# grantneale/kafka-lag-based-assignor

Hardware: AMD Instinct MI355X
Metric: partition-assignments/sec (whole node) (higher is better)
Workload: dtype int64

## Files before the change

kafka_lag_based_assignor_amd/csrc/la_device.h:

```cpp
#pragma once
#include <hip/hip_runtime.h>
#include <stdint.h>

namespace la {

constexpr int kWave = 64;

struct Rec {
    uint32_t hi, lo, tb;
};

__device__ __forceinline__ bool rec_less(const Rec& a, const Rec& b) {
    const uint64_t ka = ((uint64_t)a.hi << 32) | a.lo;
    const uint64_t kb = ((uint64_t)b.hi << 32) | b.lo;
    return (ka < kb) | ((ka == kb) & (a.tb < b.tb));
}

__device__ __forceinline__ int64_t partition_lag(int64_t begin, int64_t end, int64_t committed,
                                                 bool reset_latest) {
    const int64_t next = committed >= 0 ? committed : (reset_latest ? end : begin);
    const int64_t d = (int64_t)((uint64_t)end - (uint64_t)next);
    return d > 0 ? d : 0;
}

// ... 15 lines not shown
        return (uint32_t)__builtin_amdgcn_mov_dpp((int)x, 0x128, 0xF, 0xF, false);
    } else if constexpr (J == 16) {
        auto r = __builtin_amdgcn_permlane16_swap(x, x, false, false);
        return (__lane_id() & 16) ? r[0] : r[1];
    } else {
        auto r = __builtin_amdgcn_permlane32_swap(x, x, false, false);
        return (__lane_id() & 32) ? r[0] : r[1];
    }
}

template <int J>
__device__ __forceinline__ Rec shfl_xor(const Rec& r) {
    Rec o;
    o.hi = shfl_xor<J>(r.hi);
    o.lo = shfl_xor<J>(r.lo);
    o.tb = shfl_xor<J>(r.tb);
    return o;
}

__device__ __forceinline__ Rec shfl_xor_dyn(const Rec& r, int j) {
    switch (j) {
        case 1: return shfl_xor<1>(r);
        case 2: return shfl_xor<2>(r);
        case 4: return shfl_xor<4>(r);
        case 8: return shfl_xor<8>(r);
        case 16: return shfl_xor<16>(r);
        default: return shfl_xor<32>(r);
    }
}

template <int J>
__device__ __forceinline__ void cmpx_lanes(Rec& mine, bool keep_min) {
    const Rec o = shfl_xor<J>(mine);
    const bool take = (rec_less(o, mine) == keep_min);
    mine.hi = take ? o.hi : mine.hi;
    mine.lo = take ? o.lo : mine.lo;
    mine.tb = take ? o.tb : mine.tb;
}

__device__ __forceinline__ void cmpx_lanes_dyn(Rec& mine, int j, bool keep_min) {
    const Rec o = shfl_xor_dyn(mine, j);
    const bool take = (rec_less(o, mine) == keep_min);
    mine.hi = take ? o.hi : mine.hi;
    mine.lo = take ? o.lo : mine.lo;
    mine.tb = take ? o.tb : mine.tb;
}

__device__ __forceinline__ void cmpx_regs(Rec& a, Rec& b, bool asc) {
    const bool sw = (rec_less(b, a) == asc);
    const Rec ta = a, tb_ = b;
    a.hi = sw ? tb_.hi : ta.hi;  a.lo = sw ? tb_.lo : ta.lo;  a.tb = sw ? tb_.tb : ta.tb;
    b.hi = sw ? ta.hi : tb_.hi;  b.lo = sw ? ta.lo : tb_.lo;  b.tb = sw ? ta.tb : tb_.tb;
}

template <int L, int E, int K, int J>
__device__ __forceinline__ void bitonic_stage(Rec (&rec)[E], int gl) {
    constexpr int N = L * E;
    if constexpr (J >= E) {
        constexpr int JL = J / E;
        const bool lower = (gl & JL) == 0;
        const bool asc = (K == N) ? true : ((gl & (K / E)) == 0);
        const bool keep_min = (lower == asc);
#pragma unroll
        for (int r = 0; r < E; ++r) cmpx_lanes<JL>(rec[r], keep_min);
    } else {
#pragma unroll
        for (int r = 0; r < E; ++r) {
            if ((r & J) == 0) {
                bool asc;
                if constexpr (K == N) asc = true;
                else if constexpr (K < E) asc = ((r & K) == 0);
                else asc = ((gl & (K / E)) == 0);
                cmpx_regs(rec[r], rec[r | J], asc);
            }
        }
    }
}

template <int L, int E, int K, int J>
__device__ __forceinline__ void bitonic_merge(Rec (&rec)[E], int gl) {
    bitonic_stage<L, E, K, J>(rec, gl);
    if constexpr (J > 1) bitonic_merge<L, E, K, J / 2>(rec, gl);
}

template <int L, int E, int K = 2>
__device__ __forceinline__ void bitonic_sort_tile(Rec (&rec)[E], int gl) {
    if constexpr (L * E >= 2) {
        bitonic_merge<L, E, K, K / 2>(rec, gl);
        if constexpr (K < L * E) bitonic_sort_tile<L, E, K * 2>(rec, gl);
    }
}

__device__ __forceinline__ void bitonic_sort_lanes(Rec& rec, int gl, int n) {
    for (int k = 2; k <= n; k <<= 1) {
        for (int j = k >> 1; j > 0; j >>= 1) {
            const bool keep_min = (((gl & j) == 0) == ((gl & k) == 0));
            cmpx_lanes_dyn(rec, j, keep_min);
        }
    }
}


__device__ __forceinline__ uint32_t dpp_row_mirror(uint32_t x) {
    return (uint32_t)__builtin_amdgcn_mov_dpp((int)x, 0x140, 0xF, 0xF, false);
}

template <int M>
__device__ __forceinline__ uint32_t shfl_mirror(uint32_t x) {
    static_assert(M == 2 || M == 4 || M == 8 || M == 16 || M == 32 || M == 64, "bad mirror width");
    if constexpr (M == 2) return shfl_xor<1>(x);
    else if constexpr (M == 4) return (uint32_t)__builtin_amdgcn_mov_dpp((int)x, 0x1B, 0xF, 0xF, false);
    else if constexpr (M == 8) return (uint32_t)__builtin_amdgcn_mov_dpp((int)x, 0x141, 0xF, 0xF, false);
    else if constexpr (M == 16) return dpp_row_mirror(x);
    else if constexpr (M == 32) return shfl_xor<16>(dpp_row_mirror(x));
    else return shfl_xor<32>(shfl_xor<16>(dpp_row_mirror(x)));
}

__device__ __forceinline__ uint32_t wave_or_u32(uint32_t v) {
    v |= shfl_xor<1>(v);
    v |= shfl_xor<2>(v);
    v |= shfl_xor<4>(v);
    v |= shfl_xor<8>(v);
    v |= shfl_xor<16>(v);
    v |= shfl_xor<32>(v);
    return v;
}

__device__ __forceinline__ void wave_lds_fence() {
    __builtin_amdgcn_fence(__ATOMIC_RELEASE, "wavefront");
    __builtin_amdgcn_wave_barrier();
    __builtin_amdgcn_fence(__ATOMIC_ACQUIRE, "wavefront");
}

__device__ __forceinline__ void lds_barrier() {
    asm volatile("s_waitcnt lgkmcnt(0)\n\ts_barrier" ::: "memory");
}

__device__ __forceinline__ uint32_t wave_incl_scan_u32(uint32_t v) {
    v += (uint32_t)__builtin_amdgcn_update_dpp(0, (int)v, 0x111, 0xF, 0xF, false);
    v += (uint32_t)__builtin_amdgcn_update_dpp(0, (int)v, 0x112, 0xF, 0xF, false);
    v += (uint32_t)__builtin_amdgcn_update_dpp(0, (int)v, 0x114, 0xF, 0xF, false);
    v += (uint32_t)__builtin_amdgcn_update_dpp(0, (int)v, 0x118, 0xF, 0xF, false);
    v += (uint32_t)__builtin_amdgcn_update_dpp(0, (int)v, 0x142, 0xA, 0xF, false);
    v += (uint32_t)__builtin_amdgcn_update_dpp(0, (int)v, 0x143, 0xC, 0xF, false);
    return v;
}

__device__ __forceinline__ int wave_max_i32(int v) {
#pragma unroll
    for (int d = 32; d >= 1; d >>= 1) v = max(v, __shfl_xor(v, d));
    return v;
}

}
```

kafka_lag_based_assignor_amd/csrc/la_sort64.h:

```cpp
#pragma once
#include <hip/hip_runtime.h>
#include <stdint.h>

#include "la_device.h"

namespace la {

struct P64 {
    uint32_t lo, hi;
};

__device__ __forceinline__ P64 p64_from(uint64_t x) { P64 p; p.lo = (uint32_t)x; p.hi = (uint32_t)(x >> 32); return p; }
__device__ __forceinline__ uint64_t p64_value(const P64& p) { return ((uint64_t)p.hi << 32) | p.lo; }

template <int J>
struct KeepMin {
    static_assert(J == 1 || J == 2 || J == 4 || J == 8 || J == 16 || J == 32, "bad lane bit");
    static constexpr uint64_t value = J == 1 ? 0x5555555555555555ull : J == 2 ? 0x3333333333333333ull
                                    : J == 4 ? 0x0F0F0F0F0F0F0F0Full : J == 8 ? 0x00FF00FF00FF00FFull
                                    : J == 16 ? 0x0000FFFF0000FFFFull : 0x00000000FFFFFFFFull;
};

#define LA_DPP_TAIL " row_mask:0xf bank_mask:0xf"
#define LA_FIX_S(K) "s_xor_b64 vcc, vcc, " K "\n\t"
// ... 99 lines not shown
                 "v_cndmask_b32 %0, %3, %0, vcc\n\t"             \
                 "v_cndmask_b32 %1, %4, %1, vcc"                 \
                 : "+v"(r.lo), "+v"(r.hi), "=&v"(t)              \
                 : "v"(o.lo), "v"(o.hi), KC(KV)                  \
                 : "vcc", "scc")
template <int J, bool VO = false>
__device__ __forceinline__ void select_minmax(P64& r, const P64& o) {
    uint32_t t;
    if constexpr (VO) {
        const uint32_t kvec = keep_vec<J>();
        LA_SELECT_ASM(LA_FIX_V("%2", "%5"), "v", kvec);
    } else {
        const uint64_t keep = KeepMin<J>::value;
        LA_SELECT_ASM(LA_FIX_S("%5"), "s", keep);
    }
}

template <int M, int PAD, bool VO = false>
__device__ __forceinline__ void cmpx_same_mirror(P64& r) {
    static_assert(M == 2 || M == 4 || M == 8 || M == 16 || M == 32 || M == 64, "bad mirror width");
    if constexpr (M == 2) {
        cmpx_same_xor<1, PAD, VO>(r);
    } else if constexpr (M == 4 || M == 8 || M == 16) {
        [[maybe_unused]] const uint64_t keep = KeepMin<M / 2>::value;
        [[maybe_unused]] const uint32_t kvec = keep_vec<M / 2>();
        uint32_t t;
        if constexpr (M == 4) LA_SAME_PADS("quad_perm:[3,2,1,0]");
        else if constexpr (M == 8) LA_SAME_PADS("row_half_mirror");
        else LA_SAME_PADS("row_mirror");
    } else {
        asm volatile("s_nop 1" : "+v"(r.lo), "+v"(r.hi));
        P64 o;
        o.lo = shfl_mirror<M>(r.lo);
        o.hi = shfl_mirror<M>(r.hi);
        select_minmax<M / 2, VO>(r, o);
    }
}

#define LA_CROSS_ASM(PADSTR, CTRL, FIX, KC, KV)                                             \
    asm volatile(PADSTR                                                                     \
                 "v_sub_co_u32_dpp %2, vcc, %0, %5 " CTRL LA_DPP_TAIL "\n\t"                  \
                 "v_subb_co_u32_dpp %2, vcc, %1, %6, vcc " CTRL LA_DPP_TAIL "\n\t"            \
                 FIX                                                                        \
                 "v_cndmask_b32_dpp %3, %0, %5, vcc " CTRL LA_DPP_TAIL "\n\t"                 \
                 "v_cndmask_b32_dpp %4, %1, %6, vcc " CTRL LA_DPP_TAIL "\n\t"                 \
                 "v_sub_co_u32_dpp %2, vcc, %5, %0 " CTRL LA_DPP_TAIL "\n\t"                  \
                 "v_subb_co_u32_dpp %2, vcc, %6, %1, vcc " CTRL LA_DPP_TAIL "\n\t"            \
                 FIX                                                                        \
                 "v_cndmask_b32_dpp %0, %5, %0, vcc " CTRL LA_DPP_TAIL "\n\t"                 \
                 "v_cndmask_b32_dpp %1, %6, %1, vcc " CTRL LA_DPP_TAIL                        \
                 : "+v"(q.lo), "+v"(q.hi), "=&v"(t), "=&v"(n.lo), "=&v"(n.hi)                       \
                 : "v"(r.lo), "v"(r.hi), KC(KV)                                             \
                 : "vcc", "scc")
#define LA_CROSS_VO(PADSTR, CTRL)                                                          \
    do {                                                                                   \
        if constexpr (VO) LA_CROSS_ASM(PADSTR, CTRL, LA_FIX_V("%2", "%7"), "v", kvec);     \
        else LA_CROSS_ASM(PADSTR, CTRL, LA_FIX_S("%7"), "s", keep);                        \
    } while (0)

#define LA_CROSS_PADS(CTRL)                                   \
    do {                                                      \
        if constexpr (PAD == 0) LA_CROSS_VO(LA_PAD0, CTRL);    \
        else if constexpr (PAD == 1) LA_CROSS_VO(LA_PAD1, CTRL); \
        else LA_CROSS_VO(LA_PAD2, CTRL);                       \
    } while (0)

template <int M, int PAD, bool VO = false>
__device__ __forceinline__ void cmpx_cross_mirror(P64& r, P64& q) {
    static_assert(M == 2 || M == 4 || M == 8 || M == 16 || M == 32 || M == 64, "bad mirror width");
    [[maybe_unused]] const uint64_t keep = KeepMin<M / 2>::value;
    [[maybe_unused]] const uint32_t kvec = keep_vec<M / 2>();
    if constexpr (M <= 16) {
        uint32_t t;
        P64 n;
        if constexpr (M == 2) LA_CROSS_PADS("quad_perm:[1,0,3,2]");
        else if constexpr (M == 4) LA_CROSS_PADS("quad_perm:[3,2,1,0]");
        else if constexpr (M == 8) LA_CROSS_PADS("row_half_mirror");
        else LA_CROSS_PADS("row_mirror");
        r = n;
    } else {
        asm volatile("s_nop 1" : "+v"(r.lo), "+v"(r.hi), "+v"(q.lo), "+v"(q.hi));
        P64 oq, orr;
        oq.lo = shfl_mirror<M>(q.lo); oq.hi = shfl_mirror<M>(q.hi);
        orr.lo = shfl_mirror<M>(r.lo); orr.hi = shfl_mirror<M>(r.hi);
        select_minmax<M / 2, VO>(r, oq);
        select_minmax<M / 2, VO>(q, orr);
    }
}

__device__ __forceinline__ void cmpx_regs_p64(P64& a, P64& b) {
    uint32_t t;
    P64 n;
    asm volatile("v_sub_co_u32 %2, vcc, %0, %5\n\t"
                 "v_subb_co_u32 %2, vcc, %1, %6, vcc\n\t"
                 "v_cndmask_b32 %3, %5, %0, vcc\n\t"
                 "v_cndmask_b32 %4, %6, %1, vcc\n\t"
                 "v_cndmask_b32 %0, %0, %5, vcc\n\t"
                 "v_cndmask_b32 %1, %1, %6, vcc"
                 : "+v"(b.lo), "+v"(b.hi), "=&v"(t), "=&v"(n.lo), "=&v"(n.hi)
                 : "v"(a.lo), "v"(a.hi)
                 : "vcc", "scc");
    a = n;
}


template <int L, int E, int J, bool FIRST, bool VO = false>
__device__ __forceinline__ void clean_p64(P64 (&rec)[E]) {
    if constexpr (J >= 1) {
        if constexpr (J >= E) {
            constexpr int PADN = (E <= 2) ? 1 : 0;
#pragma unroll
            for (int r = 0; r < E; ++r) cmpx_same_xor<J / E, PADN, VO>(rec[r]);
        } else {
#pragma unroll
            for (int r = 0; r < E; ++r)
                if ((r & J) == 0) cmpx_regs_p64(rec[r], rec[r | J]);
        }
        clean_p64<L, E, J / 2, false, VO>(rec);
    }
}

template <int L, int E, int K, bool FIRST, bool VO = false>
__device__ __forceinline__ void merge_p64(P64 (&rec)[E]) {
    if constexpr (K <= L * E) {
        if constexpr (K <= E) {
#pragma unroll
            for (int r = 0; r < E; ++r)
                if ((r & (K >> 1)) == 0) cmpx_regs_p64(rec[r], rec[r ^ (K - 1)]);
        } else {
            constexpr int M = K / E;
            if constexpr (E == 1) {
                cmpx_same_mirror<M, FIRST ? 2 : 1, VO>(rec[0]);
            } else {
                constexpr int PADN = FIRST ? 2 : ((E <= 2) ? 1 : 0);
#pragma unroll
                for (int r = E / 2 - 1; r >= 0; --r) cmpx_cross_mirror<M, PADN, VO>(rec[r], rec[E - 1 - r]);
            }
        }
        clean_p64<L, E, K / 4, false, VO>(rec);
        merge_p64<L, E, K * 2, false, VO>(rec);
    }
}

template <int L, int E, bool VO = false>
__device__ __forceinline__ void bitonic_sort_tile_p64(P64 (&rec)[E]) {
    if constexpr (E == 1) merge_p64<L, E, 2, true, VO>(rec);
    else merge_p64<L, E, 2, false, VO>(rec);
}


__device__ __forceinline__ uint64_t p64_of_prev_lane(const P64& r) {
    const uint32_t lo = (uint32_t)__builtin_amdgcn_update_dpp(0, (int)r.lo, 0x138, 0xF, 0xF, false);
    const uint32_t hi = (uint32_t)__builtin_amdgcn_update_dpp(0, (int)r.hi, 0x138, 0xF, 0xF, false);
    return ((uint64_t)hi << 32) | lo;
}

__device__ __forceinline__ bool lanes_in_order_p64(const P64& r, int gl) {
    const uint64_t prev = p64_of_prev_lane(r);
    const bool bad = (gl > 0) & (prev > p64_value(r));
    return __builtin_amdgcn_ballot_w64(bad) == 0;
}

template <int L, bool VO = false>
__device__ __forceinline__ void bitonic_sort_lanes_p64(P64& rec) {
    P64 r1[1] = {rec};
    merge_p64<L, 1, 2, true, VO>(r1);
    rec = r1[0];
}

#define LA_R_STEP(CTRL, KEEP)                                                         \
    "v_sub_co_u32_dpp %[t], vcc, %[lo], %[lo] " CTRL LA_DPP_TAIL "\n\t"               \
    "v_subb_co_u32_dpp %[t], vcc, %[hi], %[hi], vcc " CTRL LA_DPP_TAIL "\n\t"         \
    "v_xor_b32 %[t], %[" KEEP "], %[t]\n\t"                                          \
    "v_cmp_gt_i32 vcc, 0, %[t]\n\t"                                                  \
    "v_cndmask_b32_dpp %[lo], %[lo], %[lo], vcc " CTRL LA_DPP_TAIL "\n\t"             \
    "v_cndmask_b32_dpp %[hi], %[hi], %[hi], vcc " CTRL LA_DPP_TAIL "\n\t"
#define LA_R_STEP_X4(KEEP)                                                                     \
    "v_mov_b32_dpp %[u], %[lo] row_half_mirror" LA_DPP_TAIL "\n\t"                               \
    "v_mov_b32_dpp %[w], %[hi] row_half_mirror" LA_DPP_TAIL "\n\t"                               \
    "s_nop 0\n\t"                                                                              \
    "v_sub_co_u32_dpp %[t], vcc, %[u], %[lo] quad_perm:[3,2,1,0]" LA_DPP_TAIL "\n\t"             \
    "v_subb_co_u32_dpp %[t], vcc, %[w], %[hi], vcc quad_perm:[3,2,1,0]" LA_DPP_TAIL "\n\t"       \
    "v_xor_b32 %[t], %[" KEEP "], %[t]\n\t"                                                   \
    "v_cmp_gt_i32 vcc, 0, %[t]\n\t"                                                           \
    "v_cndmask_b32_dpp %[lo], %[u], %[lo], vcc quad_perm:[3,2,1,0]" LA_DPP_TAIL "\n\t"           \
    "v_cndmask_b32_dpp %[hi], %[w], %[hi], vcc quad_perm:[3,2,1,0]" LA_DPP_TAIL "\n\t"
#define LA_R_X1 "quad_perm:[1,0,3,2]"
#define LA_R_X2 "quad_perm:[2,3,0,1]"
#define LA_R_M4 "quad_perm:[3,2,1,0]"
#define LA_R_NOP "s_nop 0\n\t"
#define LA_R_ADV "v_add_u32 %[sb], %[stride], %[sb]\n\t"
#define LA_R_CLAMP "v_min_u32 %[abn], %[zb], %[sb]\n\t"
#define LA_R_READ "ds_read_b64 %[nxt], %[abn]\n\t"
#define LA_R_TAIL                                            \
    "s_waitcnt lgkmcnt(0)\n\t"                               \
    "v_add_co_u32 %[lo], vcc, %[clo], %[lo]\n\t"             \
    "v_addc_co_u32 %[hi], vcc, %[chi], %[hi], vcc\n\t"       \
    "v_and_b32 %[won], %[mk], %[lo]\n\t"                     \
    "ds_write_b32 %[abc], %[won]"
#define LA_R_NET2 LA_R_STEP(LA_R_X1, "k1")
#define LA_R_NET4_REST LA_R_STEP(LA_R_M4, "k2") LA_R_CLAMP LA_R_STEP(LA_R_X1, "k1")
#define LA_R_NET8_REST LA_R_STEP("row_half_mirror", "k4") LA_R_NOP LA_R_STEP(LA_R_X2, "k2") LA_R_NOP LA_R_STEP(LA_R_X1, "k1")
#define LA_R_NET16_REST \
    LA_R_STEP("row_mirror", "k8") LA_R_NOP LA_R_STEP_X4("k4") LA_R_NOP LA_R_STEP(LA_R_X2, "k2") LA_R_NOP LA_R_STEP(LA_R_X1, "k1")
#define LA_ROUND_ASM(BODY)                                                                                             \
    asm volatile(BODY LA_R_TAIL                                                                                        \
                 : [lo] "+v"(bin.lo), [hi] "+v"(bin.hi), [sb] "+v"(sb), [abn] "=&v"(ab_next), [nxt] "=&v"(nxt),         \
                   [t] "=&v"(t), [u] "=&v"(u), [w] "=&v"(w), [won] "=&v"(won)                                           \
                 : [abc] "v"(ab_cur), [clo] "v"((uint32_t)cur), [chi] "v"((uint32_t)(cur >> 32)), [stride] "s"(stride), \
                   [zb] "s"(zb), [mk] "v"(lane_mask), [k1] "v"(kv[0]), [k2] "v"(kv[1]), [k4] "v"(kv[2]), [k8] "v"(kv[3]) \
                 : "vcc", "memory")

constexpr uint64_t kRoundSentinel = 0x7FFFFFFFFFFFFFFFull;

__device__ __forceinline__ void round_keep_vectors(int lane, uint32_t (&kv)[4]) {
#pragma unroll
    for (int b = 0; b < 4; ++b) kv[b] = (lane & (1 << b)) ? 0u : 0xFFFFFFFFu;
}

template <int L>
__device__ __forceinline__ void greedy_round_p64(P64& bin, uint32_t& sb, uint32_t ab_cur, uint32_t& ab_next, uint64_t cur,
                                                 uint64_t& nxt, uint32_t stride, uint32_t zb, uint32_t lane_mask,
                                                 const uint32_t (&kv)[4]) {
    static_assert(L == 2 || L == 4 || L == 8 || L == 16, "one statement per width up to a DPP row");
    uint32_t t, u, w, won;
    if constexpr (L == 2) LA_ROUND_ASM(LA_R_ADV LA_R_CLAMP LA_R_READ LA_R_NET2);
    else if constexpr (L == 4) LA_ROUND_ASM(LA_R_ADV LA_R_NET2 LA_R_CLAMP LA_R_STEP(LA_R_M4, "k2") LA_R_READ LA_R_STEP(LA_R_X1, "k1"));
    else if constexpr (L == 8) LA_ROUND_ASM(LA_R_NET2 LA_R_ADV LA_R_NET4_REST LA_R_READ LA_R_NET8_REST);
    else LA_ROUND_ASM(LA_R_NET2 LA_R_ADV LA_R_NET4_REST LA_R_READ LA_R_NET8_REST LA_R_NOP LA_R_NET16_REST);
}

}
```

kafka_lag_based_assignor_amd/csrc/la_wave_tile_impl.h:

```cpp
#pragma once
#include "la_kernels.h"
#include "la_device.h"
#include "la_sort64.h"
#include "la_sort32.h"
#include "la_group_small.h"
#ifdef LA_LAB
#include <cstdio>
#include <cstdlib>
#endif

namespace la {

enum : int { kModeAuto = 0, kModeWide = 1, kModeArgmin = 2 };

#ifndef LA_ABLATE
#define LA_ABLATE 0
#endif
constexpr int kAblate = LA_ABLATE;
#ifndef LA_SKIP_SORTED_ROUNDS
#define LA_SKIP_SORTED_ROUNDS 1
#endif
constexpr bool kSkipSortedRounds = LA_SKIP_SORTED_ROUNDS != 0;
#ifndef LA_WPB
#define LA_WPB 4
// ... 94 lines not shown
#pragma unroll
    for (int k = 0; k < NP; ++k) {
        const auto g = clamped_index<L, E, FULL>(a, d, 2 * k, gl);
        if constexpr (E >= 2) {
            raw.en[k] = load_at<I64x2>(src_en, g);
            raw.id[k] = load_at<I32x2>(a.pid, g);
        } else {
            raw.en[k].x = load_at<int64_t>(src_en, g); raw.en[k].y = 0;
            raw.id[k].x = load_at<int32_t>(a.pid, g); raw.id[k].y = 0;
        }
    }
}

template <int L, int E>
__device__ __forceinline__ bool second_stage_needed(const TileArgs& a) {
    return !a.lag && !a.reset_latest && a.begin;
}

template <int L, int E, bool FULL = false, typename D>
__device__ __forceinline__ void issue_begin_loads(const TileArgs& a, const D& d, int gl, Raw<E>& raw) {
    if constexpr (kAblate == 2) return;
    constexpr int NP = (E + 1) / 2;
    if (!second_stage_needed<L, E>(a)) return;
    {
        bool any = false;
#pragma unroll
        for (int k = 0; k < NP; ++k) any |= (raw.cm[k].x < 0) | (E >= 2 && raw.cm[k].y < 0);
        if (__builtin_amdgcn_ballot_w64(any) == 0 && !(a.flags & kTileAlwaysStage2)) return;
    }
#pragma unroll
    for (int k = 0; k < NP; ++k) {
        const auto g = clamped_index<L, E, FULL>(a, d, 2 * k, gl);
        using G = decltype(g);
        const bool nx = raw.cm[k].x < 0;
        if constexpr (E >= 2) {
            const bool ny = raw.cm[k].y < 0;
            const I64x2 bv = load_at<I64x2>(a.begin, (nx | ny) ? g : (G)0);
            raw.cm[k].x = nx ? bv.x : raw.cm[k].x;
            raw.cm[k].y = ny ? bv.y : raw.cm[k].y;
        } else {
            const int64_t vx = a.begin[nx ? g : (G)0];
            raw.cm[k].x = nx ? vx : raw.cm[k].x;
        }
    }
}

template <int L, int E, bool FULL = false, typename D>
__device__ __forceinline__ void finish_lags(const TileArgs& a, const D& d, int gl, const Raw<E>& raw,
                                            int64_t (&lag)[E], int32_t (&pid)[E]) {
    const bool latest = a.reset_latest != 0;
    if constexpr (kAblate == 2) {
#pragma unroll
        for (int v = 0; v < E; ++v) {
            const uint32_t h = ((uint32_t)d.p0 + (uint32_t)(v * L + gl)) * 2654435761u;
            lag[v] = (int64_t)(h >> 2) + a.reset_latest;
            pid[v] = (int32_t)((v * L + gl) * 77 + 13) & (L * E - 1);
        }
        return;
    }
    constexpr int NP = (E + 1) / 2;
    const bool cm_is_next = second_stage_needed<L, E>(a);
    auto lag_of = [&](int64_t en, int64_t cm) -> int64_t {
        if (a.lag) return en;
        if (cm_is_next) { const int64_t dlt = (int64_t)((uint64_t)en - (uint64_t)cm); return dlt > 0 ? dlt : 0; }
        return partition_lag(0, en, cm, latest);
    };
#pragma unroll
    for (int k = 0; k < NP; ++k) {
        const int e = load_index<L, E>(2 * k, gl);
        const bool shifted = !FULL && (E >= 2) && (d.p0 + (decltype(d.p0))e == (decltype(d.p0))(a.n_total - 1));
        const int64_t en_x = shifted ? raw.en[k].y : raw.en[k].x;
        const int64_t cm_x = shifted ? raw.cm[k].y : raw.cm[k].x;
        pid[2 * k] = shifted ? raw.id[k].y : raw.id[k].x;
        lag[2 * k] = lag_of(en_x, cm_x);
        if constexpr (E >= 2) {
            pid[2 * k + 1] = raw.id[k].y;
            lag[2 * k + 1] = lag_of(raw.en[k].y, raw.cm[k].y);
        }
    }
    if constexpr (FULL) return;
#pragma unroll
    for (int v = 0; v < E; ++v) {
        const bool valid = load_index<L, E>(v, gl) < d.P;
        lag[v] = valid ? lag[v] : 0;
        pid[v] = valid ? pid[v] : 0;
    }
}

template <int L, int E, bool FULL = false>
__device__ __forceinline__ void pack_records(int P, int gl, const int64_t (&lag)[E], const int32_t (&pid)[E], int sh,
                                             uint64_t lag_max, P64 (&rec)[E]) {
#pragma unroll
    for (int v = 0; v < E; ++v) {
        const int e = load_index<L, E>(v, gl);
        rec[v] = p64_from((FULL || e < P) ? (((lag_max - (uint64_t)lag[v]) << sh) | (uint32_t)pid[v]) : ~0ull);
    }
}

template <int L, int E, bool FULL = false>
__device__ __forceinline__ void sort_into_slice(uint64_t* slice, int gl, P64 (&rec)[E], int lbw, int sh) {
    using Cfg = TileCfg<L, E>;
    if constexpr (kAblate == 1 || kAblate == 4) {
#pragma unroll
        for (int r = 0; r < E; ++r) slice[slot_of(gl * E + r)] = p64_value(rec[r]);
        return;
    }
#ifdef LA_TILE_SORT64
    bitonic_sort_tile_p64<L, E>(rec);
#pragma unroll
    for (int r = 0; r < E; ++r) slice[slot_of(gl * E + r)] = p64_value(rec[r]);
    return;
#endif
    const bool by_id = sh <= Cfg::kLog2Cap;
    const int idx_bits = by_id ? sh : Cfg::kLog2Cap;
    const uint32_t idx_mask = (1u << idx_bits) - 1;
    const int top_bits = by_id ? lbw : lbw + sh;
    const int keep = 31 - idx_bits;
    const int drop = (by_id ? sh : 0) + (top_bits > keep ? top_bits - keep : 0);
    uint32_t key[E];
    if (by_id && drop == sh) {
#pragma unroll
        for (int v = 0; v < E; ++v) key[v] = (!FULL && rec[v].hi == 0xFFFFFFFFu) ? 0xFFFFFFFFu : rec[v].lo;
        bitonic_sort_tile_u32<L, E>(key);
#pragma unroll
        for (int r = 0; r < E; ++r)
            slice[slot_of(gl * E + r)] = (!FULL && key[r] == 0xFFFFFFFFu) ? ~0ull : (uint64_t)key[r];
        return;
    }
#pragma unroll
    for (int v = 0; v < E; ++v) {
        const uint64_t r = p64_value(rec[v]);
        const bool valid = FULL || r != ~0ull;
        const uint32_t idx = by_id ? ((uint32_t)r & idx_mask) : (uint32_t)load_index<L, E>(v, gl);
        if (valid) slice[slot_of((int)idx)] = r;
        key[v] = valid ? (((uint32_t)(r >> drop) << idx_bits) | idx) : 0xFFFFFFFFu;
    }
    wave_lds_fence();
    bitonic_sort_tile_u32<L, E>(key);

    P64 got[E];
#pragma unroll
    for (int r = 0; r < E; ++r) {
        const uint64_t x = slice[slot_of((int)(key[r] & idx_mask))];
        got[r] = p64_from((!FULL && key[r] == 0xFFFFFFFFu) ? ~0ull : x);
    }
    bool bad = false;
#pragma unroll
    for (int r = 0; r + 1 < E; ++r) {
        const uint64_t x = p64_value(got[r]), y = p64_value(got[r + 1]);
        bad |= (x >= y) && (FULL || y != ~0ull);
    }
    {
        const uint64_t x = p64_value(got[E - 1]);
        const uint64_t y = ((uint64_t)(uint32_t)__shfl_down((int)got[0].hi, 1) << 32) | (uint32_t)__shfl_down((int)got[0].lo, 1);
        bad |= (gl != L - 1) && (x >= y) && (FULL || y != ~0ull);
    }
    wave_lds_fence();
    if (__builtin_amdgcn_ballot_w64(bad) != 0) {
        bitonic_sort_tile_p64<L, E>(rec);
#pragma unroll
        for (int r = 0; r < E; ++r) slice[slot_of(gl * E + r)] = p64_value(rec[r]);
    } else {
#pragma unroll
        for (int r = 0; r < E; ++r) slice[slot_of(gl * E + r)] = p64_value(got[r]);
    }
}

template <int L, int LC>
__device__ __forceinline__ void greedy_rounds_tile(P64& bin, uint64_t* slice, int P, int C, int gl, int sh,
                                                   uint64_t lag_max, uint32_t pid_mask, int max_rounds) {
    for (int q = 0; q < max_rounds; ++q) {
        if (q >= 1 && kSkipSortedRounds && lanes_in_order_p64(bin, gl)) {
        } else if (q == 1) {
            bool mirrored = false;
            if constexpr (LC == L) {
                const uint64_t mine = p64_value(bin);
                const uint64_t prev = ((uint64_t)(uint32_t)__shfl_up((int)bin.hi, 1) << 32) | (uint32_t)__shfl_up((int)bin.lo, 1);
                const bool bad = (C != L) || (gl > 0 && !((prev >> 6) > (mine >> 6)));
                if (__builtin_amdgcn_ballot_w64(bad) == 0) {
                    bin.lo = shfl_mirror<L>(bin.lo);
                    bin.hi = shfl_mirror<L>(bin.hi);
                    mirrored = true;
                }
            }
            if (!mirrored) bitonic_sort_lanes_p64<LC>(bin);
        } else if (q > 1) {
            bitonic_sort_lanes_p64<LC>(bin);
        }
        const int s = q * C + gl;
        if (gl < C && s < P) {
            const uint64_t r = slice[slot_of(s)];
            const uint64_t nb = p64_value(bin) + ((lag_max - (r >> sh)) << 6);
            bin = p64_from(nb);
            slice[slot_of(s)] = ((uint64_t)(bin.lo & 63u) << 32) | ((uint32_t)r & pid_mask);
        }
    }
}

__device__ __forceinline__ uint32_t wire_element(int32_t id, int32_t rank, int id_bits, uint32_t limit, bool& bad) {
    const uint32_t r1 = (uint32_t)rank + 1u;
    const uint32_t w = (r1 << id_bits) | (uint32_t)id;
    bad |= ((uint32_t)id >> id_bits) != 0 || r1 >= limit;
    return w;
}

template <int L, int E, bool FULL = false, bool WIRE = false, typename IDX>
__device__ __forceinline__ void assign_packed(const TileArgs& a, uint64_t* slice, int32_t* rank_tab, IDX p0,
                                              IDX c0, int P, int C, int gl, int sh, uint64_t lag_max,
                                              int32_t my_rank) {
    const uint32_t pid_mask = (uint32_t)((1ull << sh) - 1);

    if (gl < C) rank_tab[gl] = my_rank;
    wave_lds_fence();

    P64 bin = p64_from((gl < C) ? (uint64_t)gl : ~0ull);
    const int rounds = (C > 0) ? (P + C - 1) / C : 0;
    int max_rounds = __builtin_amdgcn_readfirstlane(wave_max_i32(rounds));
    if constexpr (kAblate == 1 || kAblate == 3) max_rounds = 0;
    if constexpr (kAblate >= 10) max_rounds = max_rounds < kAblate - 10 ? max_rounds : kAblate - 10;
    const int c_max = __builtin_amdgcn_readfirstlane(wave_max_i32(C));
    bool done = false;
    if constexpr (L > 4) if (!done && c_max <= 4) { greedy_rounds_tile<L, 4>(bin, slice, P, C, gl, sh, lag_max, pid_mask, max_rounds); done = true; }
    if constexpr (L > 8) if (!done && c_max <= 8) { greedy_rounds_tile<L, 8>(bin, slice, P, C, gl, sh, lag_max, pid_mask, max_rounds); done = true; }
    if constexpr (L > 16) if (!done && c_max <= 16) { greedy_rounds_tile<L, 16>(bin, slice, P, C, gl, sh, lag_max, pid_mask, max_rounds); done = true; }
    if constexpr (L > 32) if (!done && c_max <= 32) { greedy_rounds_tile<L, 32>(bin, slice, P, C, gl, sh, lag_max, pid_mask, max_rounds); done = true; }
    if (!done) greedy_rounds_tile<L, L>(bin, slice, P, C, gl, sh, lag_max, pid_mask, max_rounds);
    wave_lds_fence();

    if (a.out_total && gl < C) a.out_total[c0 + (bin.lo & 63u)] = (int64_t)(p64_value(bin) >> 6);
    if constexpr (WIRE) {
        const int id_bits = a.wire_id_bits;
        const bool two = a.wire_bytes == 2;
        const int rank_bits = (two ? 16 : 32) - id_bits;
        const uint32_t limit = rank_bits >= 32 ? 0xFFFFFFFFu : (1u << rank_bits);
        bool bad = false;
        if constexpr (E >= 4) {
#pragma unroll
            for (int k = 0; k < E / 4; ++k) {
                const int s0 = k * 4 * L + 4 * gl;
                uint32_t wv[4];
#pragma unroll
                for (int i = 0; i < 4; ++i) {
                    const uint64_t w = slice[slot_of(s0 + i)];
                    bool b1 = false;
                    wv[i] = wire_element((int32_t)((uint32_t)w & pid_mask), (C > 0) ? rank_tab[(uint32_t)(w >> 32) & 63u] : -1, id_bits, limit,
                                         b1);
                    bad |= b1 && (FULL || s0 + i < P);
                }
                if (FULL || s0 + 3 < P) {
                    if (two) {
                        typedef uint32_t U32x2w __attribute__((ext_vector_type(2), aligned(2)));
                        const U32x2w v = {wv[0] | (wv[1] << 16), wv[2] | (wv[3] << 16)};
                        __builtin_nontemporal_store(v, reinterpret_cast<U32x2w*>(reinterpret_cast<uint16_t*>(a.out_wire) + p0 + s0));
                    } else {
                        typedef uint32_t U32x4w __attribute__((ext_vector_type(4), aligned(4)));
                        const U32x4w v = {wv[0], wv[1], wv[2], wv[3]};
                        __builtin_nontemporal_store(v, reinterpret_cast<U32x4w*>(reinterpret_cast<uint32_t*>(a.out_wire) + p0 + s0));
                    }
                } else {
#pragma unroll
                    for (int i = 0; i < 4; ++i)
                        if (s0 + i < P) {
                            if (two) reinterpret_cast<uint16_t*>(a.out_wire)[p0 + s0 + i] = (uint16_t)wv[i];
                            else reinterpret_cast<uint32_t*>(a.out_wire)[p0 + s0 + i] = wv[i];
                        }
                }
            }
        } else {
#pragma unroll
            for (int v = 0; v < E; ++v) {
                const int s = v * L + gl;
                if (s < P) {
                    const uint64_t w = slice[slot_of(s)];
                    const uint32_t x = wire_element((int32_t)((uint32_t)w & pid_mask), (C > 0) ? rank_tab[(uint32_t)(w >> 32) & 63u] : -1, id_bits,
                                                    limit, bad);
                    if (two) reinterpret_cast<uint16_t*>(a.out_wire)[p0 + s] = (uint16_t)x;
                    else reinterpret_cast<uint32_t*>(a.out_wire)[p0 + s] = x;
                }
            }
        }
        if (__builtin_amdgcn_ballot_w64(bad) != 0 && (threadIdx.x & (kWave - 1)) == 0) atomicOr(a.status, kStatusWire);
        return;
    }
    if constexpr (E >= 4) {
#pragma unroll
        for (int k = 0; k < E / 4; ++k) {
            const int s0 = k * 4 * L + 4 * gl;
            int32_t op[4], om[4];
#pragma unroll
            for (int i = 0; i < 4; ++i) {
                const uint64_t w = slice[slot_of(s0 + i)];
                op[i] = (int32_t)((uint32_t)w & pid_mask);
                om[i] = (C > 0) ? rank_tab[(uint32_t)(w >> 32) & 63u] : -1;
            }
            if (kAblate == 2 && (op[0] ^ om[1] ^ op[2] ^ om[3]) != 0x7FFFFFF1) continue;
            if (FULL || s0 + 3 < P) {
                typedef int I32x4 __attribute__((ext_vector_type(4), aligned(4)));
                const I32x4 vp = {op[0], op[1], op[2], op[3]}, vm = {om[0], om[1], om[2], om[3]};
                __builtin_nontemporal_store(vp, reinterpret_cast<I32x4*>(a.out_pid + p0 + s0));
                __builtin_nontemporal_store(vm, reinterpret_cast<I32x4*>(a.out_rank + p0 + s0));
            } else {
#pragma unroll
                for (int i = 0; i < 4; ++i)
                    if (s0 + i < P) { a.out_pid[p0 + s0 + i] = op[i]; a.out_rank[p0 + s0 + i] = om[i]; }
            }
        }
    } else {
#pragma unroll
        for (int v = 0; v < E; ++v) {
            const int s = v * L + gl;
            if (s < P) {
                const uint64_t w = slice[slot_of(s)];
                a.out_pid[p0 + s] = (int32_t)((uint32_t)w & pid_mask);
                a.out_rank[p0 + s] = (C > 0) ? rank_tab[(uint32_t)(w >> 32) & 63u] : -1;
            }
        }
    }
}

template <int L, int E, bool ARGMIN>
__device__ __forceinline__ void assign_wide(const TileArgs& a, uint64_t* slice, int64_t p0, int64_t c0, int P, int C,
                                            int gl, const int64_t (&lag)[E], const int32_t (&pid)[E]) {
    Rec rec[E];
#pragma unroll
    for (int v = 0; v < E; ++v) {
        const int e = load_index<L, E>(v, gl);
        rec[v].hi = rec[v].lo = rec[v].tb = 0xFFFFFFFFu;
        if (e < P) {
            const uint64_t key = (uint64_t)lag[v] ^ kLagKeyFlip;
            rec[v].hi = (uint32_t)(key >> 32);
            rec[v].lo = (uint32_t)key;
            rec[v].tb = (uint32_t)pid[v] ^ kPidBias;
        }
    }

    bitonic_sort_tile<L, E>(rec, gl);

#pragma unroll
    for (int r = 0; r < E; ++r) slice[slot_of(gl * E + r)] = rec[r].tb ^ kPidBias;
    wave_lds_fence();
#pragma unroll
    for (int v = 0; v < E; ++v) {
        const int s = v * L + gl;
        if (s < P) a.out_pid[p0 + s] = (int32_t)(uint32_t)slice[slot_of(s)];
    }
    wave_lds_fence();
#pragma unroll
    for (int r = 0; r < E; ++r) {
        const uint64_t key = ((uint64_t)rec[r].hi << 32) | rec[r].lo;
        slice[slot_of(gl * E + r)] = key ^ kLagKeyFlip;
    }
    wave_lds_fence();

    Rec bin;
    uint64_t total = kTotalBias;
    bin.tb = (gl < C) ? (uint32_t)gl : 0xFFFFFFFFu;
    if constexpr (!ARGMIN) {
        const int rounds = (C > 0) ? (P + C - 1) / C : 0;
        const int max_rounds = __builtin_amdgcn_readfirstlane(wave_max_i32(rounds));
        bin.hi = (gl < C) ? (uint32_t)(total >> 32) : 0xFFFFFFFFu;
        bin.lo = (gl < C) ? (uint32_t)total : 0xFFFFFFFFu;
        const int c_max = __builtin_amdgcn_readfirstlane(wave_max_i32(C));
        const int lc_w = c_max <= 1 ? 1 : 1 << (32 - __builtin_clz((unsigned)(c_max - 1)));
        for (int q = 0; q < max_rounds; ++q) {
            if (q > 0) bitonic_sort_lanes(bin, gl, lc_w);
            const int s = q * C + gl;
            if (gl < C && s < P) {
                const uint64_t lg = slice[slot_of(s)];
                uint64_t t = (((uint64_t)bin.hi << 32) | bin.lo) + lg;
                bin.hi = (uint32_t)(t >> 32);
                bin.lo = (uint32_t)t;
                slice[slot_of(s)] = bin.tb;
            }
        }
        total = ((uint64_t)bin.hi << 32) | bin.lo;
    } else {
        const int maxP = __builtin_amdgcn_readfirstlane(wave_max_i32(C > 0 ? P : 0));
        uint32_t count = (gl < C) ? 0u : 0xFFFFFFFFu;
        for (int s = 0; s < maxP; ++s) {
            uint32_t bc = count, bh = (uint32_t)(total >> 32), bl = (uint32_t)total, bi = bin.tb;
            for (int j = 1; j < L; j <<= 1) {
                Rec o; o.hi = bh; o.lo = bl; o.tb = bi;
                o = shfl_xor_dyn(o, j);
                Rec m; m.hi = bh; m.lo = bl; m.tb = bi;
                const uint32_t oc = (uint32_t)__shfl_xor((int)bc, j);
                const bool take = (oc < bc) | ((oc == bc) & rec_less(o, m));
                bc = take ? oc : bc; bh = take ? o.hi : bh; bl = take ? o.lo : bl; bi = take ? o.tb : bi;
            }
            if (s < P && C > 0 && bi == (uint32_t)gl) {
                total += slice[slot_of(s)];
                count += 1;
                slice[slot_of(s)] = (uint64_t)gl;
            }
        }
    }
    wave_lds_fence();

    if (a.out_total && bin.tb < (uint32_t)C)
        a.out_total[c0 + bin.tb] = (int64_t)(total ^ kTotalBias);
#pragma unroll
    for (int v = 0; v < E; ++v) {
        const int s = v * L + gl;
        if (s < P) {
            int32_t m = -1;
            if (C > 0) m = a.cons_rank[c0 + (uint32_t)slice[slot_of(s)]];
            a.out_rank[p0 + s] = m;
        }
    }
}

struct DescWords {
    int64_t p0, p1, c0, c1;
    bool exists;
};

template <int L, int E>
__device__ __forceinline__ DescWords fetch_desc(const TileArgs& a, int64_t t, int64_t n_tiles, int grp) {
    using Cfg = TileCfg<L, E>;
    const int64_t topic = t * Cfg::kGroupsPerWave + grp;
    DescWords w;
    w.exists = t < n_tiles && topic < a.n_topics;
    int64_t tc = w.exists ? topic : a.n_topics - 1;
    if (a.topic_list) tc = a.topic_list[tc];
    w.p0 = a.part_off[tc]; w.p1 = a.part_off[tc + 1];
    w.c0 = a.cons_off[tc]; w.c1 = a.cons_off[tc + 1];
    return w;
}

template <int L, int E, typename IDX = int64_t>
__device__ __forceinline__ TopicDescT<IDX> make_desc(const TileArgs& a, const DescWords& w, int gl) {
    using Cfg = TileCfg<L, E>;
    TopicDescT<IDX> d;
    d.p0 = (IDX)w.p0;
    d.c0 = (IDX)w.c0;
    const int64_t Pl = w.p1 - w.p0, Cl = w.c1 - w.c0;
    const bool bad = Pl > Cfg::kCap || Cl > L || Pl < 0 || Cl < 0;
    if (w.exists && bad && gl == 0 && !(a.flags & kTileSkipOversize)) atomicOr(a.status, kStatusShape);
    d.P = (w.exists && !bad) ? (int)Pl : 0;
    d.C = (w.exists && !bad) ? (int)Cl : 0;
    return d;
}

template <int L, int E, typename IDX = int64_t>
__device__ __forceinline__ TopicDescT<IDX> load_desc(const TileArgs& a, int64_t t, int64_t n_tiles, int grp, int gl) {
    return make_desc<L, E, IDX>(a, fetch_desc<L, E>(a, t, n_tiles, grp), gl);
}

template <int L, int E, typename IDX, bool INLINE_WIDE, bool FULL, bool WIRE = false>
__device__ __forceinline__ void packed_tile(const TileArgs& a, const TopicDescT<IDX>& cur, uint64_t* slice, int32_t* rank_tab,
                                            int64_t tile, int gl, int lane) {
    using Cfg = TileCfg<L, E>;
    Raw<E> raw;
    issue_loads<L, E, FULL>(a, cur, gl, raw);
    int32_t my_rank = 0;
    if constexpr (kAblate != 2) {
        const IDX want = cur.c0 + (IDX)gl, last = (IDX)(a.k_total > 0 ? a.k_total - 1 : 0);
        if (a.k_total > 0) my_rank = load_at<int32_t>(a.cons_rank, want < last ? want : last);
    }
    issue_begin_loads<L, E, FULL>(a, cur, gl, raw);

    P64 rec[E];
    int sh, lbw;
    bool fits;
    uint64_t lag_max;
    int64_t lag[E];
    int32_t pid[E];
    {
        finish_lags<L, E, FULL>(a, cur, gl, raw, lag, pid);
        uint32_t id_or = 0;
        uint64_t lag_or = 0;
#pragma unroll
        for (int v = 0; v < E; ++v) { id_or |= (uint32_t)pid[v]; lag_or |= (uint64_t)lag[v]; }
        id_or = (uint32_t)__builtin_amdgcn_readfirstlane((int)wave_or_u32(id_or));
        sh = 32 - __builtin_clz(id_or | 1u);
        const uint32_t hi = (uint32_t)(lag_or >> 32), lo = (uint32_t)lag_or;
        const int my_bits = hi ? 64 - __builtin_clz(hi) : (lo ? 32 - __builtin_clz(lo) : 0);
        lbw = __builtin_amdgcn_readfirstlane(wave_max_i32(my_bits));
        int lim = 63 - sh;
        if (lim > 57 - Cfg::kLog2Cap) lim = 57 - Cfg::kLog2Cap;
        fits = sh < 32 && lbw <= lim;
        lag_max = lbw >= 64 ? ~0ull : (((uint64_t)1 << lbw) - 1);
        if (fits) pack_records<L, E, FULL>(cur.P, gl, lag, pid, sh, lag_max, rec);
    }
    if (fits) {
        sort_into_slice<L, E, FULL>(slice, gl, rec, lbw, sh);
        assign_packed<L, E, FULL, WIRE>(a, slice, rank_tab, cur.p0, cur.c0, cur.P, cur.C, gl, sh, lag_max, my_rank);
    } else if constexpr (INLINE_WIDE) {
        assign_wide<L, E, false>(a, slice, (int64_t)cur.p0, (int64_t)cur.c0, cur.P, cur.C, gl, lag, pid);
    } else if (lane == 0) {
        if (a.flags & kTileNoDefer) atomicOr(a.status, kStatusBounds);
        else a.defer_list[atomicAdd(a.defer_count, 1)] = (int32_t)tile;
    }
}

__device__ __forceinline__ void tile_tail(const TileTail& t, const uint32_t* status) {
    __shared__ uint32_t s_start[kTailGroupM];
    __shared__ int32_t s_in[7 * kSmallGroupN];
    __shared__ uint32_t s_wsum[LA_WPB];
    __shared__ uint32_t s_turn, s_last;
    __threadfence_system();
    __syncthreads();
    if (threadIdx.x == 0) {
        const uint32_t done = __hip_atomic_fetch_add(t.counter, 1u, __ATOMIC_ACQ_REL, __HIP_MEMORY_SCOPE_AGENT);
        s_last = done == gridDim.x - 1 ? 1u : 0u;
    }
    __syncthreads();
    if (!s_last) return;
    __builtin_amdgcn_fence(__ATOMIC_ACQUIRE, "agent");
    if (threadIdx.x == 0) __hip_atomic_store(t.counter, 0u, __ATOMIC_RELAXED, __HIP_MEMORY_SCOPE_AGENT);
    if (t.member_off)
        group_small_body_staged<kWave * LA_WPB, kTailGroupM>(t.n, t.n_members, t.n_topics, t.part_off, t.out_pid, t.out_rank,
                                                             t.member_off, t.grouped_topic, t.grouped_partition, nullptr, s_start,
                                                             s_wsum, &s_turn, s_in, s_in + kSmallGroupN, s_in + 2 * kSmallGroupN,
                                                             s_in + 3 * kSmallGroupN, s_in + 4 * kSmallGroupN,
                                                             reinterpret_cast<uint32_t*>(s_in + 5 * kSmallGroupN),
                                                             reinterpret_cast<uint32_t*>(s_in + 6 * kSmallGroupN));
    __threadfence_system();
    __syncthreads();
    if (threadIdx.x == 0) {
        const uint32_t st = __hip_atomic_load(status, __ATOMIC_RELAXED, __HIP_MEMORY_SCOPE_AGENT);
        __hip_atomic_store(t.fin_flag, 0x80000000u | st, __ATOMIC_RELEASE, __HIP_MEMORY_SCOPE_SYSTEM);
    }
}

#ifdef LA_WPE
#define LA_WPE_ATTR __attribute__((amdgpu_waves_per_eu(LA_WPE, LA_WPE)))
#else
#define LA_WPE_ATTR
#endif
template <int L, int E, typename IDX, bool INLINE_WIDE, bool WIRE = false>
__global__ __launch_bounds__(256) LA_WPE_ATTR void wave_tile_packed_kernel(TileArgs a) {
    using Cfg = TileCfg<L, E>;
    __shared__ uint64_t lds[Cfg::kTopicsPerBlock * Cfg::kSlots];
    __shared__ int32_t rank_lds[Cfg::kTopicsPerBlock * L];

    const int lane = threadIdx.x & (kWave - 1);
    const int wave = threadIdx.x >> 6;
    const int gl = lane & (L - 1);
    const int grp = lane / L;
    uint64_t* slice = lds + (wave * Cfg::kGroupsPerWave + grp) * Cfg::kSlots;
    int32_t* rank_tab = rank_lds + (wave * Cfg::kGroupsPerWave + grp) * L;

    const int64_t n_tiles = (a.n_topics + Cfg::kGroupsPerWave - 1) / Cfg::kGroupsPerWave;
    const int64_t tile = (int64_t)blockIdx.x * Cfg::kWavesPerBlock + wave;
    if constexpr (INLINE_WIDE) {
        if (blockIdx.x == 0 && threadIdx.x == 0) *a.defer_count_next = 0;
        if (tile < n_tiles) {
            const TopicDescT<IDX> cur = load_desc<L, E, IDX>(a, tile, n_tiles, grp, gl);
            packed_tile<L, E, IDX, true, false>(a, cur, slice, rank_tab, tile, gl, lane);
        }
        if (a.tail.enabled) tile_tail(a.tail, a.status);
        return;
    }
    if (tile >= n_tiles) return;
    const TopicDescT<IDX> cur = load_desc<L, E, IDX>(a, tile, n_tiles, grp, gl);
    if constexpr (!INLINE_WIDE) {
        if (__builtin_amdgcn_ballot_w64(cur.P != Cfg::kCap || (int64_t)cur.p0 + Cfg::kCap > a.n_total) == 0) {
            packed_tile<L, E, IDX, false, true, WIRE>(a, cur, slice, rank_tab, tile, gl, lane);
            return;
        }
    }
    packed_tile<L, E, IDX, INLINE_WIDE, false, WIRE>(a, cur, slice, rank_tab, tile, gl, lane);
}

template <int L, int E, bool ARGMIN>
__global__ __launch_bounds__(256) void wave_tile_wide_kernel(TileArgs a, int from_list) {
    using Cfg = TileCfg<L, E>;
    __shared__ uint64_t lds[Cfg::kTopicsPerBlock * Cfg::kSlots];

    const int lane = threadIdx.x & (kWave - 1);
    const int wave = threadIdx.x >> 6;
    const int gl = lane & (L - 1);
    const int grp = lane / L;
    uint64_t* slice = lds + (wave * Cfg::kGroupsPerWave + grp) * Cfg::kSlots;

    const int64_t n_tiles = (a.n_topics + Cfg::kGroupsPerWave - 1) / Cfg::kGroupsPerWave;
    const int64_t n_waves = (int64_t)gridDim.x * Cfg::kWavesPerBlock;
    const int64_t count = from_list ? (int64_t)*a.defer_count : n_tiles;
    if (from_list && blockIdx.x == 0 && threadIdx.x == 0) *a.defer_count_next = 0;
    for (int64_t i = (int64_t)blockIdx.x * Cfg::kWavesPerBlock + wave; i < count; i += n_waves) {
        const int64_t tile = from_list ? (int64_t)a.defer_list[i] : i;
        const TopicDesc d = load_desc<L, E>(a, tile, n_tiles, grp, gl);
        Raw<E> raw;
        issue_loads<L, E>(a, d, gl, raw);
        issue_begin_loads<L, E>(a, d, gl, raw);
        int64_t lag[E];
        int32_t pid[E];
        finish_lags<L, E>(a, d, gl, raw, lag, pid);
        assign_wide<L, E, ARGMIN>(a, slice, d.p0, d.c0, d.P, d.C, gl, lag, pid);
        wave_lds_fence();
    }
}

template <typename K>
static hipError_t resident_blocks(K kernel, int threads, int* out) {
    int dev = 0, cus = 0, per_cu = 0;
    hipError_t e;
    if ((e = hipGetDevice(&dev)) != hipSuccess) return e;
    if ((e = hipDeviceGetAttribute(&cus, hipDeviceAttributeMultiprocessorCount, dev)) != hipSuccess) return e;
    if ((e = hipOccupancyMaxActiveBlocksPerMultiprocessor(&per_cu, kernel, threads, 0)) != hipSuccess) return e;
    if (per_cu < 1) per_cu = 1;
    *out = cus * per_cu;
    return hipSuccess;
}

template <int L, int E>
static hipError_t launch_one(const TileArgs& a_in, int mode, hipStream_t stream, bool* tail_done) {
    TileArgs a = a_in;
    const bool want_tail = a.tail.enabled != 0;
    a.tail.enabled = 0;
    using Cfg = TileCfg<L, E>;
    const int64_t blocks = (a.n_topics + Cfg::kTopicsPerBlock - 1) / Cfg::kTopicsPerBlock;
    if (blocks <= 0) return hipSuccess;
    struct Res { std::atomic<int> inl{0}, wide{0}, argmin{0}; };
    static Res s_res[33];
    hipError_t e;
    int dev = 0;
    if ((e = hipGetDevice(&dev)) != hipSuccess) return e;
    const bool cached = dev >= 0 && dev < 32;
    Res& rs = s_res[cached ? dev : 32];
    std::atomic<int>&s_inline = rs.inl, &s_wide = rs.wide, &s_argmin = rs.argmin;
    int res_inline = cached ? s_inline.load(std::memory_order_acquire) : 0, res_wide = s_wide.load(std::memory_order_relaxed),
        res_argmin = s_argmin.load(std::memory_order_relaxed);
    if (res_inline == 0) {
        if ((e = resident_blocks(wave_tile_packed_kernel<L, E, uint32_t, true>, Cfg::kThreads, &res_inline)) != hipSuccess) return e;
        if ((e = resident_blocks(wave_tile_wide_kernel<L, E, false>, Cfg::kThreads, &res_wide)) != hipSuccess) return e;
        if ((e = resident_blocks(wave_tile_wide_kernel<L, E, true>, Cfg::kThreads, &res_argmin)) != hipSuccess) return e;
        if (cached) {
            s_wide.store(res_wide, std::memory_order_relaxed);
            s_argmin.store(res_argmin, std::memory_order_relaxed);
            s_inline.store(res_inline, std::memory_order_release);
        }
#ifdef LA_LAB
        printf("resident blocks: inline %d wide %d argmin %d (needed %lld)\n", res_inline, res_wide, res_argmin, (long long)blocks);
#endif
    }
    const dim3 b(Cfg::kThreads);
    auto grid = [&](int resident) { return dim3((unsigned)(blocks < resident ? blocks : resident)); };
    if (mode == kModeArgmin) {
        LA_LAUNCH((wave_tile_wide_kernel<L, E, true>), grid(res_argmin), b, 0, stream, a, 0);
    } else if (mode == kModeWide) {
        LA_LAUNCH((wave_tile_wide_kernel<L, E, false>), grid(res_wide), b, 0, stream, a, 0);
    } else {
        if (!a.defer_count || !a.defer_count_next || !a.defer_list) return hipErrorInvalidValue;
        const bool idx32 = a.n_total < ((int64_t)1 << 29) && a.k_total < ((int64_t)1 << 30) && !(a.flags & 1);
        if (idx32 && blocks <= res_inline && !(a.flags & 2) && !(a.flags & kTileWireOut)) {
            if (want_tail && tail_done) {
                a.tail.enabled = 1;
                *tail_done = true;
            }
            LA_LAUNCH((wave_tile_packed_kernel<L, E, uint32_t, true>), dim3((unsigned)blocks), b, 0, stream, a);
            return hipGetLastError();
        }
        if (a.flags & kTileWireOut) {
            if (!idx32 || !(a.flags & kTileNoDefer) || !a.out_wire) return hipErrorInvalidValue;
            LA_LAUNCH((wave_tile_packed_kernel<L, E, uint32_t, false, true>), dim3((unsigned)blocks), b, 0, stream, a);
            return hipGetLastError();
        }
        if (idx32)
            LA_LAUNCH((wave_tile_packed_kernel<L, E, uint32_t, false>), dim3((unsigned)blocks), b, 0, stream, a);
        else
            LA_LAUNCH((wave_tile_packed_kernel<L, E, int64_t, false>), dim3((unsigned)blocks), b, 0, stream, a);
        if (a.flags & kTileNoDefer) return hipGetLastError();
#ifdef LA_LAB
        if (getenv("LA_NO_WIDE")) return hipGetLastError();
#endif
        LA_LAUNCH((wave_tile_wide_kernel<L, E, false>), grid(res_wide), b, 0, stream, a, 1);
    }
    return hipGetLastError();
}

template <int L>
static inline hipError_t launch_l(int e, const TileArgs& a, int mode, hipStream_t stream, bool* tail_done) {
    switch (e) {
        case 1: return launch_one<L, 1>(a, mode, stream, tail_done);
        case 2: return launch_one<L, 2>(a, mode, stream, tail_done);
        case 4: return launch_one<L, 4>(a, mode, stream, tail_done);
        case 8: return launch_one<L, 8>(a, mode, stream, tail_done);
        default: return launch_one<L, 16>(a, mode, stream, tail_done);
    }
}

}
```

Before: 187.2 billion.

## Use scalar loads and readlane-based wave reductions in packed tile path

Replaces cross-lane shuffle-based reductions (wave_or, wave_max) with DPP row reductions followed by scalar readlanes, and exploits per-group uniformity to compute maxima via readlane over group leaders. Topic descriptor offsets are loaded through the constant address space so the compiler can use scalar loads, with a per-lane select by group. __shfl_up/down are replaced by DPP row shifts, and the wave index is made scalar. The intent is to cut VALU/LDS shuffle latency in the per-tile prologue, at the cost of relying on value uniformity within groups and on DPP row-shift boundary semantics.

Measured after the change: 190.6 billion (median of 6 runs). 1.02x the previous value.

```diff
diff --git a/kafka_lag_based_assignor_amd/csrc/la_device.h b/kafka_lag_based_assignor_amd/csrc/la_device.h
--- a/kafka_lag_based_assignor_amd/csrc/la_device.h
+++ b/kafka_lag_based_assignor_amd/csrc/la_device.h
@@ -191,4 +191,29 @@
     return v;
 }
 
-}
+
+__device__ __forceinline__ uint32_t wave_or_u32_uniform(uint32_t v) {
+    v |= shfl_xor<1>(v);
+    v |= shfl_xor<2>(v);
+    v |= shfl_xor<4>(v);
+    v |= shfl_xor<8>(v);
+    return (uint32_t)__builtin_amdgcn_readlane((int)v, 0) | (uint32_t)__builtin_amdgcn_readlane((int)v, 16) |
+           (uint32_t)__builtin_amdgcn_readlane((int)v, 32) | (uint32_t)__builtin_amdgcn_readlane((int)v, 48);
+}
+
+template <int L>
+__device__ __forceinline__ int wave_max_of_groups_i32(int v) {
+    int m = __builtin_amdgcn_readlane(v, 0);
+#pragma unroll
+    for (int g = 1; g < kWave / L; ++g) {
+        const int x = __builtin_amdgcn_readlane(v, g * L);
+        m = x > m ? x : m;
+    }
+    return m;
+}
+
+__device__ __forceinline__ int bits_of_or_u64(uint32_t hi_or, uint32_t lo_or) {
+    return hi_or ? 64 - __builtin_clz(hi_or) : (lo_or ? 32 - __builtin_clz(lo_or) : 0);
+}
+
+}
diff --git a/kafka_lag_based_assignor_amd/csrc/la_sort64.h b/kafka_lag_based_assignor_amd/csrc/la_sort64.h
--- a/kafka_lag_based_assignor_amd/csrc/la_sort64.h
+++ b/kafka_lag_based_assignor_amd/csrc/la_sort64.h
@@ -275,6 +275,12 @@
 __device__ __forceinline__ uint64_t p64_of_prev_lane(const P64& r) {
     const uint32_t lo = (uint32_t)__builtin_amdgcn_update_dpp(0, (int)r.lo, 0x138, 0xF, 0xF, false);
     const uint32_t hi = (uint32_t)__builtin_amdgcn_update_dpp(0, (int)r.hi, 0x138, 0xF, 0xF, false);
+    return ((uint64_t)hi << 32) | lo;
+}
+
+__device__ __forceinline__ uint64_t p64_of_next_lane(const P64& r) {
+    const uint32_t lo = (uint32_t)__builtin_amdgcn_update_dpp(0, (int)r.lo, 0x130, 0xF, 0xF, false);
+    const uint32_t hi = (uint32_t)__builtin_amdgcn_update_dpp(0, (int)r.hi, 0x130, 0xF, 0xF, false);
     return ((uint64_t)hi << 32) | lo;
 }
 
diff --git a/kafka_lag_based_assignor_amd/csrc/la_wave_tile_impl.h b/kafka_lag_based_assignor_amd/csrc/la_wave_tile_impl.h
--- a/kafka_lag_based_assignor_amd/csrc/la_wave_tile_impl.h
+++ b/kafka_lag_based_assignor_amd/csrc/la_wave_tile_impl.h
@@ -270,7 +270,7 @@
     }
     {
         const uint64_t x = p64_value(got[E - 1]);
-        const uint64_t y = ((uint64_t)(uint32_t)__shfl_down((int)got[0].hi, 1) << 32) | (uint32_t)__shfl_down((int)got[0].lo, 1);
+        const uint64_t y = p64_of_next_lane(got[0]);
         bad |= (gl != L - 1) && (x >= y) && (FULL || y != ~0ull);
     }
     wave_lds_fence();
@@ -293,7 +293,7 @@
             bool mirrored = false;
             if constexpr (LC == L) {
                 const uint64_t mine = p64_value(bin);
-                const uint64_t prev = ((uint64_t)(uint32_t)__shfl_up((int)bin.hi, 1) << 32) | (uint32_t)__shfl_up((int)bin.lo, 1);
+                const uint64_t prev = p64_of_prev_lane(bin);
                 const bool bad = (C != L) || (gl > 0 && !((prev >> 6) > (mine >> 6)));
                 if (__builtin_amdgcn_ballot_w64(bad) == 0) {
                     bin.lo = shfl_mirror<L>(bin.lo);
@@ -333,10 +333,10 @@
 
     P64 bin = p64_from((gl < C) ? (uint64_t)gl : ~0ull);
     const int rounds = (C > 0) ? (P + C - 1) / C : 0;
-    int max_rounds = __builtin_amdgcn_readfirstlane(wave_max_i32(rounds));
+    int max_rounds = wave_max_of_groups_i32<L>(rounds);
     if constexpr (kAblate == 1 || kAblate == 3) max_rounds = 0;
     if constexpr (kAblate >= 10) max_rounds = max_rounds < kAblate - 10 ? max_rounds : kAblate - 10;
-    const int c_max = __builtin_amdgcn_readfirstlane(wave_max_i32(C));
+    const int c_max = wave_max_of_groups_i32<L>(C);
     bool done = false;
     if constexpr (L > 4) if (!done && c_max <= 4) { greedy_rounds_tile<L, 4>(bin, slice, P, C, gl, sh, lag_max, pid_mask, max_rounds); done = true; }
     if constexpr (L > 8) if (!done && c_max <= 8) { greedy_rounds_tile<L, 8>(bin, slice, P, C, gl, sh, lag_max, pid_mask, max_rounds); done = true; }
@@ -545,6 +545,28 @@
     return w;
 }
 
+template <int L, int E>
+__device__ __forceinline__ DescWords fetch_desc_uniform(const TileArgs& a, int64_t t, int grp) {
+    constexpr int G = TileCfg<L, E>::kGroupsPerWave;
+    typedef const int64_t __attribute__((address_space(4))) * ConstWords;
+    const ConstWords po = (ConstWords)(uintptr_t)a.part_off + t * G;
+    const ConstWords co = (ConstWords)(uintptr_t)a.cons_off + t * G;
+    int64_t pw[G + 1], cw[G + 1];
+#pragma unroll
+    for (int k = 0; k <= G; ++k) { pw[k] = po[k]; cw[k] = co[k]; }
+    DescWords w;
+    w.exists = true;
+    w.p0 = pw[0]; w.p1 = pw[1];
+    w.c0 = cw[0]; w.c1 = cw[1];
+#pragma unroll
+    for (int g = 1; g < G; ++g) {
+        const bool mine = grp >= g;
+        w.p0 = mine ? pw[g] : w.p0; w.p1 = mine ? pw[g + 1] : w.p1;
+        w.c0 = mine ? cw[g] : w.c0; w.c1 = mine ? cw[g + 1] : w.c1;
+    }
+    return w;
+}
+
 template <int L, int E, typename IDX = int64_t>
 __device__ __forceinline__ TopicDescT<IDX> make_desc(const TileArgs& a, const DescWords& w, int gl) {
     using Cfg = TileCfg<L, E>;
@@ -564,6 +586,14 @@
     return make_desc<L, E, IDX>(a, fetch_desc<L, E>(a, t, n_tiles, grp), gl);
 }
 
+template <int L, int E, typename IDX = int64_t>
+__device__ __forceinline__ TopicDescT<IDX> load_desc_uniform(const TileArgs& a, int64_t t, int64_t n_tiles, int grp, int gl) {
+    constexpr int G = TileCfg<L, E>::kGroupsPerWave;
+    if (!a.topic_list && (t + 1) * G <= a.n_topics)
+        return make_desc<L, E, IDX>(a, fetch_desc_uniform<L, E>(a, t, grp), gl);
+    return make_desc<L, E, IDX>(a, fetch_desc<L, E>(a, t, n_tiles, grp), gl);
+}
+
 template <int L, int E, typename IDX, bool INLINE_WIDE, bool FULL, bool WIRE = false>
 __device__ __forceinline__ void packed_tile(const TileArgs& a, const TopicDescT<IDX>& cur, uint64_t* slice, int32_t* rank_tab,
                                             int64_t tile, int gl, int lane) {
@@ -589,11 +619,9 @@
         uint64_t lag_or = 0;
 #pragma unroll
         for (int v = 0; v < E; ++v) { id_or |= (uint32_t)pid[v]; lag_or |= (uint64_t)lag[v]; }
-        id_or = (uint32_t)__builtin_amdgcn_readfirstlane((int)wave_or_u32(id_or));
+        id_or = wave_or_u32_uniform(id_or);
         sh = 32 - __builtin_clz(id_or | 1u);
-        const uint32_t hi = (uint32_t)(lag_or >> 32), lo = (uint32_t)lag_or;
-        const int my_bits = hi ? 64 - __builtin_clz(hi) : (lo ? 32 - __builtin_clz(lo) : 0);
-        lbw = __builtin_amdgcn_readfirstlane(wave_max_i32(my_bits));
+        lbw = bits_of_or_u64(wave_or_u32_uniform((uint32_t)(lag_or >> 32)), wave_or_u32_uniform((uint32_t)lag_or));
         int lim = 63 - sh;
         if (lim > 57 - Cfg::kLog2Cap) lim = 57 - Cfg::kLog2Cap;
         fits = sh < 32 && lbw <= lim;
@@ -653,7 +681,7 @@
     __shared__ int32_t rank_lds[Cfg::kTopicsPerBlock * L];
 
     const int lane = threadIdx.x & (kWave - 1);
-    const int wave = threadIdx.x >> 6;
+    const int wave = __builtin_amdgcn_readfirstlane((int)(threadIdx.x >> 6));
     const int gl = lane & (L - 1);
     const int grp = lane / L;
     uint64_t* slice = lds + (wave * Cfg::kGroupsPerWave + grp) * Cfg::kSlots;
@@ -664,14 +692,14 @@
     if constexpr (INLINE_WIDE) {
         if (blockIdx.x == 0 && threadIdx.x == 0) *a.defer_count_next = 0;
         if (tile < n_tiles) {
-            const TopicDescT<IDX> cur = load_desc<L, E, IDX>(a, tile, n_tiles, grp, gl);
+            const TopicDescT<IDX> cur = load_desc_uniform<L, E, IDX>(a, tile, n_tiles, grp, gl);
             packed_tile<L, E, IDX, true, false>(a, cur, slice, rank_tab, tile, gl, lane);
         }
         if (a.tail.enabled) tile_tail(a.tail, a.status);
         return;
     }
     if (tile >= n_tiles) return;
-    const TopicDescT<IDX> cur = load_desc<L, E, IDX>(a, tile, n_tiles, grp, gl);
+    const TopicDescT<IDX> cur = load_desc_uniform<L, E, IDX>(a, tile, n_tiles, grp, gl);
     if constexpr (!INLINE_WIDE) {
         if (__builtin_amdgcn_ballot_w64(cur.P != Cfg::kCap || (int64_t)cur.p0 + Cfg::kCap > a.n_total) == 0) {
             packed_tile<L, E, IDX, false, true, WIRE>(a, cur, slice, rank_tab, tile, gl, lane);
```
